# the3cloud/zktls

Hardware: AMD Instinct MI355X
Metric: trace-cells/s (higher is better)
Workload: dtype u32

## Files before the change

### zktls_amd/csrc/kernels.h

```cpp
#pragma once
#include <hip/hip_runtime.h>
#include <stddef.h>
#include <stdint.h>

#include "babybear.cuh"

namespace zk {

struct NttPassArgs {
    const uint32_t* in;
    uint32_t* out;
    uint64_t in_ld, out_ld;
    uint32_t ncols;
    uint32_t num_tiles;
    uint32_t log_m;
    uint64_t in_tile_mul, in_stride;
    uint64_t out_tile_mul, out_stride;
    uint32_t bitrev_out;
    uint32_t map_mode;
    uint64_t tile_perm;
    uint32_t fast_path;
    uint32_t debug_flags;
    uint32_t cols_per_thread;
    uint32_t bench_tag;
    const uint32_t* w1024;
    const uint32_t* pre;
    const uint32_t* post;
};
hipError_t launch_ntt_pass(const NttPassArgs& a, bool inverse, hipStream_t s);

constexpr int FUSED_COSETS = 2;
struct LdeFusedArgs {
    const uint32_t* in;
    uint64_t in_ld, out_ld;
    uint32_t ncols;
    uint32_t num_tiles;
    uint32_t map_rot;
    uint32_t grid;
    uint32_t bench_tag;
    uint64_t in_tile_mul, in_stride;
    uint64_t out_tile_mul, out_stride;
    const uint32_t* w1024_inv;
    const uint32_t* w1024_fwd;
    uint32_t* out[FUSED_COSETS];
    const uint32_t* pre[FUSED_COSETS];
    const uint32_t* post[FUSED_COSETS];
};
hipError_t launch_lde_fused(const LdeFusedArgs& a, hipStream_t s);
hipError_t launch_fused_table(uint32_t* out, const uint32_t* in, uint32_t blocks, int mode, hipStream_t s);
bool lde_fused_supported(const LdeFusedArgs& a);

struct LdeSmallArgs {
    const uint32_t* in;
    uint64_t in_ld, out_ld;
    uint32_t ncols;
    uint32_t cosets;
    uint32_t groups;
    uint32_t reserved;
    const uint32_t* tw_inv;
    const uint32_t* tw_fwd;
    uint32_t* out[16];
    const uint32_t* pre[16];
};
bool lde_small_supported(const LdeSmallArgs& a, int log_n);
hipError_t launch_lde_small(const LdeSmallArgs& a, int log_n, hipStream_t s);

struct ColPassArgs {
    const uint32_t* in;
    uint32_t* out;
    uint64_t in_batch, out_batch;
    uint32_t count;
    uint32_t tload, tstore, in_brev, out_brev;
    const uint32_t* w1024;
    const uint32_t* pre;
    const uint32_t* post2d;
};
hipError_t launch_ntt_colpass(const ColPassArgs& a, bool inverse, hipStream_t s);
hipError_t launch_post2d_table(uint32_t* out, uint32_t w, uint32_t shift, uint32_t scale, hipStream_t s);

struct CombineArgs {
    const uint32_t* in;
    uint32_t* out;
    uint64_t in_ld, out_ld;
    uint32_t ncols;
    uint64_t groups;
    int log_r;
    uint64_t in_group_mul, in_elem_mul, out_group_mul, out_elem_mul;
    int bitrev_out;
    int inverse;
    const uint32_t* tw;
};
hipError_t launch_ntt_combine(const CombineArgs& a, hipStream_t s);
hipError_t launch_combine_table(uint32_t* out, uint32_t rows, uint64_t groups, uint32_t w, uint32_t shift, uint32_t scale, int bits, hipStream_t s);

hipError_t launch_pow_table(uint32_t* out, size_t n, uint32_t base, uint32_t scale, hipStream_t s);
hipError_t launch_post_table(uint32_t* out, uint32_t rows, uint32_t cols, uint32_t omega,
                             uint32_t shift, uint32_t scale, hipStream_t s);

struct MatDesc {
    const uint32_t* ptr;
    uint64_t ld;
    uint32_t width;
};
constexpr int MAX_LEAF_MATS = 8;
constexpr uint32_t COOP_MAX_NODES = 16384;
uint32_t coop_max_nodes();
constexpr uint32_t COOP_TOP_NODES = 512;
struct LeafArgs {
    MatDesc mats[MAX_LEAF_MATS];
    int nmats;
    uint64_t height;
    uint32_t* digests;
};
hipError_t launch_hash_rows(const LeafArgs& a, hipStream_t s);
hipError_t launch_compress_level(const uint32_t* children, uint32_t* parents, uint64_t count,
                                 hipStream_t s);
hipError_t launch_inject(uint32_t* nodes, const uint32_t* extra, uint64_t count, hipStream_t s);
bool compress_inject_ok(const LeafArgs& a);
hipError_t launch_compress_inject(const uint32_t* children, const LeafArgs& a, hipStream_t s);
hipError_t launch_compress_top(uint32_t* tree, uint32_t count, hipStream_t s);
hipError_t launch_compress_sub(uint32_t* tree, uint32_t count, uint32_t sub, hipStream_t s);
hipError_t launch_hash_sub(const LeafArgs& a, uint32_t sub, hipStream_t s);
hipError_t launch_merkle_p24_colmajor(const uint32_t* mat, uint32_t cols, int log_rows, uint32_t* tree, hipStream_t s);
hipError_t launch_merkle_p24_rowmajor(const uint32_t* mat, uint64_t ld, uint32_t width, int log_rows, uint32_t* tree, hipStream_t s);
struct P2Tables;
hipError_t hash_upload_p2_tables(const P2Tables& t, hipStream_t s);
hipError_t stark_upload_p2_tables(const P2Tables& t, hipStream_t s);
namespace p2chip { struct MerkleTraceArgs; struct LayerPathsArgs; struct P2RArgs; struct MrecChainArgs; struct Fri16TranscriptArgs; }
hipError_t launch_p2chip_merkle(const p2chip::MerkleTraceArgs& a, hipStream_t s);
namespace p24chip { struct MerkleTraceArgs; struct LayerPathsArgs; struct RowPathsArgs; }
hipError_t launch_p24chip_merkle(const p24chip::MerkleTraceArgs& a, hipStream_t s);
hipError_t launch_p24chip_row_paths(const p24chip::RowPathsArgs& a, hipStream_t s);
hipError_t launch_p24chip_layer_paths(const p24chip::LayerPathsArgs& a, hipStream_t s);
hipError_t launch_fri16_transcript(const p2chip::Fri16TranscriptArgs& a, hipStream_t s);
hipError_t launch_p2chip_layer_paths(const p2chip::LayerPathsArgs& a, hipStream_t s);
hipError_t launch_mrec_chains(const p2chip::MrecChainArgs& a, hipStream_t s);
hipError_t launch_p2r_rows(const p2chip::P2RArgs& a, hipStream_t s);
hipError_t launch_permute_states(uint32_t* states, uint64_t count, hipStream_t s);

hipError_t launch_fill_uniform(uint32_t* out, uint64_t ld, uint64_t seed, uint64_t rows,
                               uint32_t width, hipStream_t s);
hipError_t launch_gen_trace(uint32_t* out, uint64_t ld, uint64_t seed, uint64_t rows,
                            uint32_t width, hipStream_t s);
hipError_t launch_gen_trace_logup(uint32_t* out, uint64_t ld, uint64_t seed, uint64_t rows, uint32_t width, uint32_t pairs,
                                  uint64_t recv_seed, uint32_t recv_width, hipStream_t s);
hipError_t launch_small_eval(const uint32_t* in, uint64_t in_ld, uint32_t* out, uint64_t out_ld, int log_n, int log_out, uint32_t width,
                             uint32_t w, uint32_t shift, uint32_t scale, int bitrev_out, hipStream_t s);
hipError_t launch_transpose(const uint32_t* in, uint32_t* out, uint64_t rows, uint64_t cols, int rev_bits_in, int rev_bits_out, hipStream_t s);
hipError_t launch_convert(const uint32_t* in, uint32_t* out, uint64_t n, bool to_monty_form,
                          hipStream_t s);

hipError_t launch_domain_tables(uint32_t* xs, uint32_t* sel_first, uint32_t* sel_last, uint32_t* itw, int log_n, int log_blowup, hipStream_t s);

struct QuotientArgs {
    const uint32_t* lde;
    uint64_t ld;
    uint32_t width;
    int log_n;
    int lanes_per_row;
    const uint32_t* xs;
    const uint32_t* sel_first;
    uint32_t wn_inv;
    uint32_t inv_zh_even, inv_zh_odd;
    const uint32_t* alpha_pow;
    uint32_t pairs;
    const uint32_t* perm;
    uint64_t perm_ld;
    Ext gamma, beta;
    Ext cumsum;
    const uint32_t* sel_last;
    uint32_t* addend_out;
    const uint32_t* addend;
    uint32_t* out;
    uint32_t* lde_out;
    uint64_t lde_ld;
};
hipError_t launch_quotient(const QuotientArgs& a, hipStream_t s);
hipError_t launch_logup_addend(const QuotientArgs& a, hipStream_t s);

constexpr uint32_t AIR_SLOT_EXTRA = 4;
constexpr uint32_t AIR_GP = 36;
#if defined(__HIPCC__)
__host__ __device__
#endif
inline uint32_t air_lds_base(uint32_t slot, uint32_t W) {
    if (slot < W) return AIR_GP * (slot >> 2) + (slot & 3u);
    if (slot < 2 * W) { const uint32_t c = slot - W; return AIR_GP * (c >> 2) + (c & 3u) + 4u; }
    const uint32_t x = slot - 2 * W;
    return AIR_GP * ((W >> 2) + (x >> 2)) + (x & 3u);
}
struct QuotientAirArgs {
    const uint32_t* lde; uint64_t ld; uint32_t width; int log_n;
    const uint32_t* xs; const uint32_t* sel_first; const uint32_t* sel_last;
    uint32_t wn_inv;
    int log_qd;
    uint32_t inv_zh[4];
    const uint32_t* body;
    uint32_t n_constraints;
    const uint32_t* weights;
    const uint32_t* pub;
    uint32_t* out;
    uint32_t* lde_out; uint64_t lde_ld;
    const uint32_t* recs; uint32_t n_terms; uint32_t n_public;
    const uint32_t* addend;
    uint32_t no_chain;
    uint32_t wide;
    uint32_t cls[6];
};
constexpr uint32_t AIR_WIDE_POINTS = 64, AIR_WIDE_PITCH = 65;
inline bool air_wide_form(uint32_t width, uint32_t n_terms, int log_n, uint32_t n_public) {
    return n_terms >= 2048 && width % 4 == 0 && (size_t)AIR_WIDE_PITCH * (width + AIR_SLOT_EXTRA + n_public) * 4 <= 160 * 1024 && log_n >= 6;
}
ZK_HD uint32_t air_wide_word(uint32_t slot, uint32_t W) {
    if (slot < W) return AIR_WIDE_PITCH * slot;
    if (slot < 2 * W) return AIR_WIDE_PITCH * (slot - W) + 1u;
    return AIR_WIDE_PITCH * (W + (slot - 2 * W));
}
hipError_t launch_quotient_air(const QuotientAirArgs& a, hipStream_t s);

hipError_t launch_inv_denominators(const uint32_t* xs, uint64_t count, const Ext& z0, const Ext& z1, int npoints,
                                   uint32_t* out, uint32_t* xw, uint64_t xw_count, hipStream_t s);

struct OpenArgs {
    const uint32_t* mat;
    uint64_t ld;
    uint32_t width;
    uint64_t rows;
    const uint32_t* xw;
    uint64_t xw_stride;
    uint32_t* partial;
    int tx;
};
size_t open_chunks(uint64_t rows, uint32_t width, uint64_t ld, const uint32_t* mat);
hipError_t launch_open(const OpenArgs& a, int npts, const Ext& scale0, const Ext& scale1, uint32_t* out, hipStream_t s);

struct ReducedArgs {
    const uint32_t* tlde; uint64_t t_ld; uint32_t width;
    const uint32_t* qlde; uint64_t q_ld; uint32_t q_width;
    const uint32_t* plde; uint64_t p_ld; uint32_t p_width;
    uint64_t rows;
    const uint32_t* alpha_pow;
    const uint32_t* dinv;
    Ext y_loc, y_next, y_pl, y_pn, y_q, off_next, off_pl, off_pn, off_q;
    Ext off_loc;
    int accumulate;
    uint32_t* out;
};
hipError_t launch_reduced_opening(const ReducedArgs& a, uint32_t* scratch_at, hipStream_t s);
int rowdot_form(uint32_t width, uint64_t rows);

struct PermArgs {
    const uint32_t* trace; uint64_t ld;
    uint64_t rows; uint32_t pairs;
    Ext gamma, beta;
    uint32_t* out; uint64_t out_ld;
};
hipError_t launch_perm_trace(const PermArgs& a, uint32_t* block_scratch, hipStream_t s);

constexpr int LOOKUP_REC_WORDS = 12;
struct LookupArgs {
    const uint32_t* table; uint32_t ni, cols;
    Ext gamma, bpow[9];
    const uint8_t* cmap; uint32_t n_used, chunk_mask;
};
constexpr uint32_t LOOKUP_MAX_COLS = 512, LOOKUP_STAGE_MAX_USED = 56;
struct MachinePermArgs {
    LookupArgs lk;
    const uint32_t* trace; uint64_t ld; uint64_t rows;
    uint32_t* out; uint64_t out_ld;
    const uint32_t* pre; uint64_t pre_ld; uint32_t pre_w;
};
bool lookup_perm_two_sources_ok(const MachinePermArgs& a);
hipError_t launch_perm_trace_machine(const MachinePermArgs& a, uint32_t* block_scratch, hipStream_t s);
struct MachineQuotArgs {
    LookupArgs lk;
    const uint32_t* lde; uint64_t ld; const uint32_t* perm; uint64_t perm_ld; int log_n;
    int log_qd;
    const uint32_t* xs; const uint32_t* sel_first; const uint32_t* sel_last; uint32_t wn_inv;
    const uint32_t* weights;
    Ext cumsum;
    uint32_t* addend;
};
hipError_t launch_lookup_addend(const MachineQuotArgs& a, hipStream_t s);

hipError_t launch_fri_fold(const uint32_t* in, uint32_t* out, const uint32_t* itw, uint64_t half, const Ext& beta, hipStream_t s);
hipError_t launch_ext_add(uint32_t* dst, const uint32_t* src, uint64_t count, hipStream_t s);
hipError_t launch_fri_fold_dev(const uint32_t* in, uint32_t* out, const uint32_t* itw, uint64_t half, const uint32_t* beta_ptr,
                               int squarings, hipStream_t s);

struct DevChallenger {
    uint32_t state[16];
    uint32_t in[8];
    uint32_t out[8];
    int32_t n_in, n_out;
};
hipError_t launch_fri_challenge(DevChallenger* chal, const uint32_t* root, uint32_t* beta_out, uint32_t* root_log, hipStream_t s);


struct GrindArgs {
    uint32_t state[16];
    int slot;
    uint32_t mask;
};
hipError_t launch_grind(const GrindArgs& a, uint32_t base, uint32_t count, uint32_t* result, hipStream_t s);

struct GatherDesc {
    const uint32_t* src;
    uint32_t dst_off;
    uint32_t nwords;
};
hipError_t launch_gather(const GatherDesc* descs, uint32_t ndesc, uint32_t* dst, hipStream_t s);

hipError_t launch_copy_bytes(void* dst, const void* src, size_t bytes, hipStream_t s);
hipError_t launch_fill_bytes(void* dst, int byte, size_t bytes, hipStream_t s);
hipError_t launch_copy2d(uint32_t* dst, uint64_t dst_ld, const uint32_t* src, uint64_t src_ld, uint32_t width, uint64_t rows, hipStream_t s);
}
```

### zktls_amd/csrc/prover.cpp

```cpp
#include <atomic>
#include <chrono>
#include <condition_variable>
#include <deque>
#include <cstring>
#include <functional>
#include <mutex>
#include <string>
#include <thread>
#include <vector>

#include "proof_common.h"
#include "batch.h"

namespace zk { std::atomic<bool> g_fri_graph{true}; }
namespace zk {

extern std::atomic<uint64_t> g_p2_generation;
void air_digest_cached(const AirView& a, uint32_t out[8]) {
    struct Entry { std::vector<uint32_t> words; uint64_t generation; uint32_t dg[8]; };
    static std::mutex mu;
    static std::vector<Entry> cache;
    const uint64_t gen = g_p2_generation.load();
    {
        std::lock_guard<std::mutex> lk(mu);
        for (const Entry& e : cache)
            if (e.generation == gen && e.words.size() == a.words && memcmp(e.words.data(), a.w, a.words * 4) == 0) { memcpy(out, e.dg, 32); return; }
    }
    air_digest(a, out);
    std::lock_guard<std::mutex> lk(mu);
    if (cache.size() >= 64) cache.erase(cache.begin());
    Entry e;
    e.words.assign(a.w, a.w + a.words);
    e.generation = gen;
    memcpy(e.dg, out, 32);
    cache.push_back(std::move(e));
}

static int ensure_domain(zkhip_ctx* ctx, int log_n, int log_blowup = 1) {
    if (ctx->dom_log_n == log_n && ctx->dom_log_blowup == log_blowup) return ZKHIP_OK;
    for (const auto& d : ctx->domains)
        if (d.log_n == log_n && d.log_blowup == log_blowup) {
            ctx->dom_xs = d.xs; ctx->dom_sel_first = d.sel_first; ctx->dom_sel_last = d.sel_last; ctx->dom_itw = d.itw;
            ctx->dom_log_n = log_n; ctx->dom_log_blowup = log_blowup;
            return ZKHIP_OK;
        }
    zkhip_ctx::DomainSet d{log_n, log_blowup, nullptr, nullptr, nullptr, nullptr};
    const size_t m = (size_t)1 << (log_n + log_blowup), mq = (size_t)1 << (log_n + (log_blowup < 2 ? log_blowup : 2));
    ZK_HIP(hipMalloc((void**)&d.xs, m * 4));
    ZK_HIP(hipMalloc((void**)&d.sel_first, mq * 4));
    ZK_HIP(hipMalloc((void**)&d.sel_last, mq * 4));
    ZK_HIP(hipMalloc((void**)&d.itw, (m / 2) * 4));
    ZK_HIP(launch_domain_tables(d.xs, d.sel_first, d.sel_last, d.itw, log_n, log_blowup, ctx->stream));
    ctx->domains.push_back(d);
    ctx->dom_xs = d.xs; ctx->dom_sel_first = d.sel_first; ctx->dom_sel_last = d.sel_last; ctx->dom_itw = d.itw;
    ctx->dom_log_n = log_n; ctx->dom_log_blowup = log_blowup;
    return ZKHIP_OK;
}
static int ensure_fold_table(zkhip_ctx* ctx, int log_h) {
    if (ctx->dom_log_n >= 0 && ctx->dom_log_n + ctx->dom_log_blowup >= log_h) return ZKHIP_OK;
    return ensure_domain(ctx, log_h - 1 < 5 ? 5 : log_h - 1, 1);
}

static int d2h(zkhip_ctx* ctx, void* dst, const void* src, size_t bytes) { return dev_d2h(ctx, dst, src, bytes); }
static int h2d(zkhip_ctx* ctx, void* dst, const void* src, size_t bytes) { return dev_h2d(ctx, dst, src, bytes); }

struct LogupIn {
    Ext cumsum = ext_zero();
    uint32_t pairs = 0;
    const uint32_t* perm_lde = nullptr;
    Ext gamma = ext_zero(), beta = ext_zero();
};
static int run_quotient(zkhip_ctx* ctx, const uint32_t* lde, size_t ld, int log_n, uint32_t width, const Ext& alpha,
                        const LogupIn& lu, uint32_t* out_chunks, uint32_t* lde_out = nullptr, size_t lde_ld = 0) {
    if (ctx->dom_log_n != log_n) ZK_TRY(ensure_domain(ctx, log_n));
    const uint32_t G = width / 4;
    const size_t K = (size_t)3 * G + (lu.pairs ? lu.pairs + 3 : 0);
    std::vector<Ext> ap(K);
    Ext w = ext_one();
    for (size_t k = K; k-- > 0;) { ap[k] = w; w = ext_mul(w, alpha); }
    std::vector<uint32_t> tab(16 * (size_t)G + 4 * (K - 3 * (size_t)G));
    for (uint32_t g = 0; g < G; g++) {
        for (int t = 0; t < 3; t++) memcpy(&tab[16 * (size_t)g + 4 * t], ap[3 * (size_t)g + t].c, 16);
        tab[16 * (size_t)g + 12] = to_monty(g + 1);
        tab[16 * (size_t)g + 13] = to_monty(2 * g + 3);
        tab[16 * (size_t)g + 14] = to_monty(5 * g + 7);
        tab[16 * (size_t)g + 15] = 0;
    }
    for (size_t k = 3 * (size_t)G; k < K; k++) memcpy(&tab[16 * (size_t)G + 4 * (k - 3 * (size_t)G)], ap[k].c, 16);
    void* d_ap;
    ZK_TRY(ctx_reserve(ctx, S_APOW_Q, tab.size() * 4, &d_ap));
    ZK_TRY(h2d(ctx, d_ap, tab.data(), tab.size() * 4));
    QuotientArgs q{};
    q.lde = lde; q.ld = ld; q.width = width; q.log_n = log_n;
    q.lanes_per_row = pow2ceil((int)G) > 16 ? 16 : pow2ceil((int)G);
    q.xs = ctx->dom_xs; q.sel_first = ctx->dom_sel_first;
    q.wn_inv = finv(two_adic_generator(log_n));
    const uint32_t gn = fpow(MONTY_GEN, (uint64_t)1 << log_n);
    q.inv_zh_even = finv(fsub(gn, MONTY_R1));
    q.inv_zh_odd = finv(fsub(fneg(gn), MONTY_R1));
    q.alpha_pow = (const uint32_t*)d_ap;
    q.pairs = lu.pairs; q.perm = lu.perm_lde; q.perm_ld = 4 * ((uint64_t)lu.pairs + 1);
    q.gamma = lu.gamma; q.beta = lu.beta; q.cumsum = lu.cumsum; q.sel_last = ctx->dom_sel_last;
    q.out = out_chunks;
    q.lde_out = lde_out; q.lde_ld = lde_ld;
    if (lu.pairs) {
        void* v_add;
        ZK_TRY(ctx_reserve(ctx, S_ADDEND, ((size_t)2 << log_n) * 16, &v_add));
        q.addend_out = (uint32_t*)v_add;
        ZK_HIP(launch_logup_addend(q, ctx->stream));
        q.addend = (const uint32_t*)v_add;
    }
    ZK_HIP(launch_quotient(q, ctx->stream));
    return ZKHIP_OK;
}

static int run_quotient_air(zkhip_ctx* ctx, const AirView& air, const uint32_t* lde, size_t ld, int log_n, uint32_t width,
                            const uint32_t* public_values, const Ext& alpha, uint32_t* out_chunks, uint32_t* lde_out, size_t lde_ld,
                            const Ext& scale = ext_one(), const uint32_t* addend = nullptr) {
    if (ctx->dom_log_n != log_n || ctx->dom_log_blowup < air.lqd) ZK_TRY(ensure_domain(ctx, log_n, air.lqd));
    std::vector<uint32_t> body, weights;
    air_device_image(air, alpha, body, weights, scale);
    std::vector<uint32_t> pub(air.n_public ? air.n_public : 1, 0u);
    for (uint32_t i = 0; i < air.n_public; i++) pub[i] = to_monty(public_values[i]);
    std::vector<uint32_t> recs;
    uint32_t cls[6] = {0, 0, 0, 0, 0, 0};
    const bool wide = !t_batcher && ld % 4 == 0 && (reinterpret_cast<uintptr_t>(lde) & 15u) == 0 &&
                      air_wide_form(width, (uint32_t)air_term_count(air), log_n, 0);
    if (wide) air_term_records_wide(air, alpha, pub.data(), recs, cls, scale);
    else air_term_records(air, alpha, pub.data(), recs, scale);
    const size_t body_w = (body.size() + 3) & ~(size_t)3, pub_w = (pub.size() + 3) & ~(size_t)3;
    std::vector<uint32_t> stage(body_w + weights.size() + pub_w + recs.size(), 0u);
    memcpy(stage.data(), body.data(), body.size() * 4);
    memcpy(stage.data() + body_w, weights.data(), weights.size() * 4);
    memcpy(stage.data() + body_w + weights.size(), pub.data(), pub.size() * 4);
    if (!recs.empty()) memcpy(stage.data() + body_w + weights.size() + pub_w, recs.data(), recs.size() * 4);
    void* d_stage;
    ZK_TRY(ctx_reserve(ctx, S_APOW_Q, stage.size() * 4, &d_stage));
    ZK_TRY(h2d(ctx, d_stage, stage.data(), stage.size() * 4));
    QuotientAirArgs q{};
    q.lde = lde; q.ld = ld; q.width = width; q.log_n = log_n;
    q.xs = ctx->dom_xs; q.sel_first = ctx->dom_sel_first; q.sel_last = ctx->dom_sel_last;
    q.wn_inv = finv(two_adic_generator(log_n));
    q.log_qd = air.lqd;
    const uint32_t gn = fpow(MONTY_GEN, (uint64_t)1 << log_n), wq = two_adic_generator(air.lqd);
    for (int j = 0; j < (1 << air.lqd); j++) q.inv_zh[j] = finv(fsub(fmul(gn, fpow(wq, (uint64_t)j)), MONTY_R1));
    q.body = (const uint32_t*)d_stage; q.n_constraints = air.K;
    q.weights = (const uint32_t*)d_stage + body_w; q.pub = (const uint32_t*)d_stage + body_w + weights.size();
    q.out = out_chunks; q.lde_out = lde_out; q.lde_ld = lde_ld;
    q.recs = recs.empty() ? nullptr : (const uint32_t*)d_stage + body_w + weights.size() + pub_w;
    q.n_terms = (uint32_t)(recs.size() / 8); q.n_public = recs.empty() ? air.n_public : 0u;
    q.wide = wide ? 1u : 0u;
    for (int i = 0; i < 6; i++) q.cls[i] = cls[i];
    q.addend = addend;
    ZK_HIP(launch_quotient_air(q, ctx->stream));
    return ZKHIP_OK;
}

static int run_open(zkhip_ctx* ctx, const uint32_t* lde, size_t ld, int log_n, uint32_t width, const Ext* z, int npts,
                    const uint32_t* xw, uint32_t* d_out) {
    const uint64_t n = (uint64_t)1 << log_n;
    OpenArgs o{};
    o.mat = lde; o.ld = ld; o.width = width; o.rows = n; o.xw = xw; o.xw_stride = n;
    o.tx = pow2ceil((int)width) > 64 ? 64 : pow2ceil((int)width);
    const size_t nchunks = open_chunks(n, width, ld, lde);
    void* part;
    ZK_TRY(ctx_reserve(ctx, S_PARTIAL, nchunks * npts * width * 16, &part));
    o.partial = (uint32_t*)part;
    Ext scale[2] = {ext_zero(), ext_zero()};
    const uint32_t ginv = finv(MONTY_GEN), ninv = finv(to_monty((uint32_t)(n % P)));
    for (int k = 0; k < npts; k++)
        scale[k] = ext_mul_base(ext_sub_base(ext_pow(ext_mul_base(z[k], ginv), n), MONTY_R1), ninv);
    ZK_HIP(launch_open(o, npts, scale[0], scale[1], d_out, ctx->stream));
    return ZKHIP_OK;
}

static int commit_hw(zkhip_ctx* ctx, const uint32_t* mat, size_t ld, uint32_t width, int log_h, uint32_t* tree, int hw) {
    if (hw == 24) { ZK_HIP(launch_merkle_p24_rowmajor(mat, ld, width, log_h, tree, ctx->stream)); return ZKHIP_OK; }
    MatDesc md{mat, ld, width};
    return op_merkle_commit(ctx, &md, 1, log_h, tree);
}

static int fri_commit_phase(zkhip_ctx* ctx, Challenger& ch, const Shape& sh, int H, int RL, uint32_t* layers, uint32_t* ltrees,
                            const std::vector<size_t>& layer_off, const std::vector<size_t>& tree_off, uint32_t* fold_tmp, size_t m,
                            const uint32_t* const* inject, uint32_t* pf, size_t& pos) {
    hipStream_t st = ctx->stream;
    const int K = sh.K;
    const size_t arity = (size_t)1 << K;
    uint32_t root[8];
#ifdef ZKHIP_AB_HOOKS
    static const bool fri_on_host = [] { const char* e = getenv("ZKHIP_FRI_HOST"); return e && atoi(e) != 0; }();
#else
    constexpr bool fri_on_host = false;
#endif
    void* v_chal = nullptr;
    uint32_t *d_betas = nullptr, *d_roots = nullptr;
    DevChallenger* d_chal = nullptr;
    if (!fri_on_host && RL > 0) {
        ZK_TRY(ctx_reserve(ctx, S_CHAL, sizeof(DevChallenger) + (size_t)RL * 12 * 4, &v_chal));
        d_chal = (DevChallenger*)v_chal;
        d_betas = (uint32_t*)((char*)v_chal + sizeof(DevChallenger));
        d_roots = d_betas + 4 * (size_t)RL;
        DevChallenger hc{};
        for (int i = 0; i < 16; i++) hc.state[i] = ch.state[i];
        for (int i = 0; i < 8; i++) { hc.in[i] = ch.in[i]; hc.out[i] = ch.out[i]; }
        hc.n_in = ch.n_in; hc.n_out = ch.n_out;
        ZK_TRY(h2d(ctx, d_chal, &hc, sizeof hc));
    }
    auto enqueue_layers = [&]() -> int {
    for (int l = 0; l < RL; l++) {
        const int lh = H - K * (l + 1);
        const size_t rows = (size_t)1 << lh;
        uint32_t* cur = layers + layer_off[l];
        uint32_t* tree = ltrees + tree_off[l];
        ZK_TRY(commit_hw(ctx, cur, 4 * arity, (uint32_t)(4 * arity), lh, tree, sh.hw));
        Ext beta = ext_zero();
        if (d_chal) {
            ZK_HIP(launch_fri_challenge(d_chal, tree + (2 * rows - 2) * 8, d_betas + 4 * l, d_roots + 8 * l, st));
        } else {
            ZK_TRY(d2h(ctx, root, tree + (2 * rows - 2) * 8, 32));
            for (int i = 0; i < 8; i++) { ch.observe(root[i]); pf[pos++] = from_monty(root[i]); }
            beta = ch.sample_ext();
        }
        const uint32_t* src = cur;
        for (int j = 0; j < K; j++) {
            const size_t out_cnt = (size_t)1 << (H - K * l - j - 1);
            uint32_t* dst = (j == K - 1) ? layers + layer_off[l + 1] : fold_tmp + ((j & 1) ? 4 * (m / 2) : 0);
            if (d_chal) ZK_HIP(launch_fri_fold_dev(src, dst, ctx->dom_itw, out_cnt, d_betas + 4 * l, j, st));
            else ZK_HIP(launch_fri_fold(src, dst, ctx->dom_itw, out_cnt, beta, st));
            src = dst;
            beta = ext_mul(beta, beta);
        }
        const int reached = H - K * (l + 1);
        if (inject && inject[reached]) ZK_HIP(launch_ext_add(layers + layer_off[l + 1], inject[reached], (uint64_t)1 << reached, st));
    }
    return ZKHIP_OK;
    };
#ifdef ZKHIP_AB_HOOKS
    static const bool env_graph = [] { const char* e = getenv("ZKHIP_FRI_GRAPH"); return !e || atoi(e) != 0; }();
    const bool use_graph = env_graph && g_fri_graph.load();
#else
    const bool use_graph = g_fri_graph.load();
#endif
    if (d_chal && use_graph && !t_batcher) {
        std::vector<uint64_t> key = {(uint64_t)H, (uint64_t)K, (uint64_t)RL, (uint64_t)sh.hw, (uint64_t)m, (uint64_t)(uintptr_t)layers,
                                     (uint64_t)(uintptr_t)ltrees, (uint64_t)(uintptr_t)fold_tmp, (uint64_t)(uintptr_t)d_chal,
                                     (uint64_t)(uintptr_t)ctx->dom_itw};
        for (size_t o : layer_off) key.push_back(o);
        for (size_t o : tree_off) key.push_back(o);
        if (inject) for (int h = 0; h <= H; h++) key.push_back((uint64_t)(uintptr_t)inject[h]);
        if (!ctx->fri_graph_exec || ctx->fri_graph_key != key) {
            if (ctx->fri_graph_exec) { (void)hipGraphExecDestroy(ctx->fri_graph_exec); ctx->fri_graph_exec = nullptr; }
            hipGraph_t graph = nullptr;
            ZK_HIP(hipStreamBeginCapture(st, hipStreamCaptureModeThreadLocal));
// ... 1240 lines not shown
```

### zktls_amd/csrc/stark.hip

```cpp
#include <atomic>

#include "poseidon2.cuh"
#include "kernels.h"
#include "batch.h"

namespace zk {

hipError_t stark_upload_p2_tables(const P2Tables& t, hipStream_t s) { return p2_upload_tables(t, s); }


ZK_D Ext ld_ext(const uint32_t* p) {
    uint4 v = *reinterpret_cast<const uint4*>(p);
    return Ext{{v.x, v.y, v.z, v.w}};
}
ZK_D void st_ext(uint32_t* p, const Ext& e) { *reinterpret_cast<uint4*>(p) = make_uint4(e.c[0], e.c[1], e.c[2], e.c[3]); }

ZK_D Ext group_sum(Ext v, int width) {
    for (int off = width >> 1; off > 0; off >>= 1) {
        Ext o;
        o.c[0] = __shfl_down(v.c[0], off, width);
        o.c[1] = __shfl_down(v.c[1], off, width);
        o.c[2] = __shfl_down(v.c[2], off, width);
        o.c[3] = __shfl_down(v.c[3], off, width);
        v = Ext{{dadd(v.c[0], o.c[0]), dadd(v.c[1], o.c[1]), dadd(v.c[2], o.c[2]), dadd(v.c[3], o.c[3])}};
    }
    return v;
}

__device__ __forceinline__ void domain_tables_kernel_body(uint32_t* xs, uint32_t* sel_first, uint32_t* sel_last, uint32_t* itw, int log_n, int log_blowup, uint32_t g_pow_n) {
    const uint32_t p = blockIdx.x * blockDim.x + threadIdx.x;
    const int H = log_n + log_blowup, lq = log_blowup < 2 ? log_blowup : 2, Hq = log_n + lq;
    if (p >= (1u << H)) return;
    const uint32_t e = __brev(p) >> (32 - H);
    const uint32_t wm = two_adic_generator(H);
    const uint32_t x = fmul(MONTY_GEN, fpow(wm, e));
    xs[p] = x;
    if (p < (1u << Hq)) {
        const uint32_t eq = __brev(p) >> (32 - Hq);
        const uint32_t xn = fmul(g_pow_n, fpow(two_adic_generator(lq), eq & ((1u << lq) - 1u)));
        const uint32_t zh = fsub(xn, MONTY_R1);
        sel_first[p] = fmul(zh, finv(fsub(x, MONTY_R1)));
        sel_last[p] = fmul(zh, finv(fsub(x, finv(two_adic_generator(log_n)))));
    }
    if (p < (1u << (H - 1))) {
        const uint32_t ei = (H > 1) ? (__brev(p) >> (32 - (H - 1))) : 0u;
        itw[p] = fmul(finv(fpow(wm, ei)), MONTY_INV2);
    }
}
__global__ void domain_tables_kernel(uint32_t* xs, uint32_t* sel_first, uint32_t* sel_last, uint32_t* itw, int log_n, int log_blowup, uint32_t g_pow_n) { domain_tables_kernel_body(xs, sel_first, sel_last, itw, log_n, log_blowup, g_pow_n); }
struct domain_tables_kernel_bargs { uint32_t* xs; uint32_t* sel_first; uint32_t* sel_last; uint32_t* itw; int log_n; int log_blowup; uint32_t g_pow_n; static domain_tables_kernel_bargs make(uint32_t* xs, uint32_t* sel_first, uint32_t* sel_last, uint32_t* itw, int log_n, int log_blowup, uint32_t g_pow_n) { return domain_tables_kernel_bargs{xs, sel_first, sel_last, itw, log_n, log_blowup, g_pow_n}; } };
__global__ void domain_tables_kernel_batch(const domain_tables_kernel_bargs* __restrict__ zk_arr) { const domain_tables_kernel_bargs& zk_b = zk_arr[blockIdx.z]; domain_tables_kernel_body(zk_b.xs, zk_b.sel_first, zk_b.sel_last, zk_b.itw, zk_b.log_n, zk_b.log_blowup, zk_b.g_pow_n); }

hipError_t launch_domain_tables(uint32_t* xs, uint32_t* sel_first, uint32_t* sel_last, uint32_t* itw, int log_n, int log_blowup, hipStream_t s) {
    const uint32_t m = 1u << (log_n + log_blowup);
    const uint32_t gpn = fpow(MONTY_GEN, (uint64_t)1 << log_n);
    ZK_LAUNCH(domain_tables_kernel, domain_tables_kernel_batch, domain_tables_kernel_bargs, dim3((m + 255) / 256), dim3(256), 0, s, xs, sel_first, sel_last, itw, log_n, log_blowup, gpn);
    return hipGetLastError();
}

typedef uint32_t u32x4_nt __attribute__((ext_vector_type(4)));
ZK_D uint4 ld_stream(const uint32_t* p) {
    const u32x4_nt v = __builtin_nontemporal_load(reinterpret_cast<const u32x4_nt*>(p));
    return make_uint4(v.x, v.y, v.z, v.w);
}
ZK_D void dacc1(uint64_t& acc, uint32_t a0, uint32_t b0) {
    const uint64_t t = dmac(a0, b0, acc);
    acc = ((uint64_t)dred((uint32_t)(t >> 32)) << 32) | (uint32_t)t;
}
template <int CTRL>
ZK_D uint32_t dpp_mov(uint32_t v) { return (uint32_t)__builtin_amdgcn_update_dpp(0, (int)v, CTRL, 0xF, 0xF, false); }
ZK_D uint32_t row_group_sum(uint32_t v, int L) {
    if (L > 1) v = dadd(v, dpp_mov<0xB1>(v));
    if (L > 2) v = dadd(v, dpp_mov<0x4E>(v));
    if (L > 4) v = dadd(v, dpp_mov<0x141>(v));
    if (L > 8) v = dadd(v, dpp_mov<0x140>(v));
    return v;
}
__device__ __forceinline__ void logup_addend_kernel_body(const QuotientArgs& a) {
    const int H = a.log_n + 1;
    const uint32_t m = 1u << H;
    const uint32_t p = blockIdx.x * blockDim.x + threadIdx.x;
    if (p >= m) return;
    const uint32_t e = __brev(p) >> (32 - H);
    const uint32_t pn = __brev((e + 2) & (m - 1)) >> (32 - H);
    const uint32_t* row = a.lde + (uint64_t)p * a.ld;
    const uint32_t* prow = a.perm + (uint64_t)p * a.perm_ld;
    const uint32_t* pnrow = a.perm + (uint64_t)pn * a.perm_ld;
    const uint32_t* wl = a.alpha_pow + 16 * (a.width / 4);
    const uint32_t sel_trans = dsub(a.xs[p], a.wn_inv);
    Ext r = ext_zero(), sphi = ext_zero(), sphin = ext_zero();
    for (uint32_t q = 0; q < a.pairs; q++) {
        const uint4 vs = *reinterpret_cast<const uint4*>(row + 8 * q);
        const uint4 vr = *reinterpret_cast<const uint4*>(row + 8 * q + 4);
        const Ext ds = ext_add(ext_add_base(a.gamma, vs.x), ext_mul_base_dev(a.beta, vs.y));
        const Ext dr = ext_add(ext_add_base(a.gamma, vr.x), ext_mul_base_dev(a.beta, vr.y));
        const Ext phi = ld_ext(prow + 4 * q), phin = ld_ext(pnrow + 4 * q);
        const Ext c = ext_sub(ext_mul_dev(ext_mul_dev(phi, ds), dr), ext_sub(dr, ds));
        r = ext_add(r, ext_mul_dev(c, ld_ext(wl + 4 * q)));
        sphi = ext_add(sphi, phi);
        sphin = ext_add(sphin, phin);
    }
    const Ext S = ld_ext(prow + 4 * a.pairs), Sn = ld_ext(pnrow + 4 * a.pairs);
    const Ext F1 = ext_mul_base_dev(ld_ext(wl + 4 * a.pairs), a.sel_first[p]);
    const Ext F2 = ext_mul_base_dev(ld_ext(wl + 4 * (a.pairs + 1)), sel_trans);
    const Ext F3 = ext_mul_base_dev(ld_ext(wl + 4 * (a.pairs + 2)), a.sel_last[p]);
    r = ext_add(r, ext_mul_dev(F1, ext_sub(S, sphi)));
    r = ext_add(r, ext_mul_dev(F2, ext_sub(ext_sub(Sn, S), sphin)));
    r = ext_add(r, ext_mul_dev(F3, ext_sub(S, a.cumsum)));
    st_ext(a.addend_out + 4 * (uint64_t)p, r);
}
__global__ void __launch_bounds__(256) logup_addend_kernel(QuotientArgs a) { logup_addend_kernel_body(a); }
struct logup_addend_kernel_bargs { QuotientArgs a; static logup_addend_kernel_bargs make(QuotientArgs a) { return logup_addend_kernel_bargs{a}; } };
__global__ void __launch_bounds__(256) logup_addend_kernel_batch(const logup_addend_kernel_bargs* __restrict__ zk_arr) { const logup_addend_kernel_bargs& zk_b = zk_arr[blockIdx.z]; logup_addend_kernel_body(zk_b.a); }

hipError_t launch_logup_addend(const QuotientArgs& a, hipStream_t s) {
    const uint64_t m = 2ull << a.log_n;
    ZK_LAUNCH(logup_addend_kernel, logup_addend_kernel_batch, logup_addend_kernel_bargs, dim3((unsigned)((m + 255) / 256)), dim3(256), 0, s, a);
    return hipGetLastError();
}
constexpr int QCHAIN = 16;
template <int NG>
#ifndef QWPE
#define QWPE 2
#endif
__device__ __forceinline__ void quotient_kernel_body(const QuotientArgs& a) {
    const int L = a.lanes_per_row;
    const uint32_t gid = blockIdx.x * blockDim.x + threadIdx.x;
    const int lane = gid % L;
    const int H = a.log_n + 1;
    const uint32_t m = 1u << H;
    const uint32_t nchains = m / QCHAIN;
    const bool live = gid / L < nchains;
    const uint32_t chain = live ? gid / L : 0u;
    const uint32_t parity = chain & 1u;
    uint32_t e = 2u * ((chain >> 1) * QCHAIN) + parity;
    const uint32_t G = a.width / 4;
    const uint32_t inv_zh = parity ? a.inv_zh_odd : a.inv_zh_even;

    uint4 cur[NG], nxt[NG];
    uint32_t p = __brev(e) >> (32 - H);
#pragma unroll
    for (int t = 0; t < NG; t++) {
        const uint32_t g = lane + L * t;
        cur[t] = g < G ? *reinterpret_cast<const uint4*>(a.lde + (uint64_t)p * a.ld + 4 * g) : make_uint4(0, 0, 0, 0);
    }
    constexpr bool HOIST = NG <= 4;
    uint4 W[HOIST ? NG : 1][4];
    if (HOIST) {
#pragma unroll
        for (int t = 0; t < NG; t++) {
            const uint32_t g = lane + L * t;
            const uint4* wp = reinterpret_cast<const uint4*>(a.alpha_pow + 16 * (g < G ? g : 0u));
#pragma unroll
            for (int i = 0; i < 4; i++) W[HOIST ? t : 0][i] = wp[i];
        }
    }
    for (int step = 0; step < QCHAIN; step++) {
        const uint32_t en = (e + 2) & (m - 1);
        const uint32_t pn = __brev(en) >> (32 - H);
#pragma unroll
        for (int t = 0; t < NG; t++) {
            const uint32_t g = lane + L * t;
            nxt[t] = g < G ? ld_stream(a.lde + (uint64_t)pn * a.ld + 4 * g) : make_uint4(0, 0, 0, 0);
        }
        const uint32_t x = a.xs[p];
        const uint32_t sel_first = a.sel_first[p];
        const uint32_t sel_trans = dsub(x, a.wn_inv);
        uint64_t acc[4] = {0, 0, 0, 0};
#pragma unroll
        for (int t = 0; t < NG; t++) {
            const uint32_t g = lane + L * t;
            if (g < G) {
                const uint4 v = cur[t];
                const uint4* wp = reinterpret_cast<const uint4*>(a.alpha_pow + 16 * g);
                const uint4 w0 = HOIST ? W[HOIST ? t : 0][0] : wp[0], w1 = HOIST ? W[HOIST ? t : 0][1] : wp[1];
                const uint4 w2 = HOIST ? W[HOIST ? t : 0][2] : wp[2], kk = HOIST ? W[HOIST ? t : 0][3] : wp[3];
                const uint32_t aab = dmul(dmont_lazy(v.x, v.x), v.y);
                const uint32_t c1 = dsub(dsub(v.z, aab), kk.x);
                const uint32_t ab = dmul(v.x, v.y);
                const uint32_t c2 = dmul(dsub_lazy(dsub(dsub(nxt[t].w, ab), v.z), kk.y), sel_trans);
                const uint32_t c3 = dmul(dsub_lazy(v.w, kk.z), sel_first);
                dacc2(acc[0], w0.x, c1, w1.x, c2); dacc1(acc[0], w2.x, c3);
                dacc2(acc[1], w0.y, c1, w1.y, c2); dacc1(acc[1], w2.y, c3);
                dacc2(acc[2], w0.z, c1, w1.z, c2); dacc1(acc[2], w2.z, c3);
                dacc2(acc[3], w0.w, c1, w1.w, c2); dacc1(acc[3], w2.w, c3);
            }
        }
        Ext r = Ext{{dacc_finish(acc[0]), dacc_finish(acc[1]), dacc_finish(acc[2]), dacc_finish(acc[3])}};
        if (a.addend && lane == 0) r = ext_add(r, ld_ext(a.addend + 4 * (uint64_t)p));
#pragma unroll
        for (int i = 0; i < 4; i++) r.c[i] = row_group_sum(r.c[i], L);
        if (lane == 0 && live) {
            r = ext_mul_base_dev(r, inv_zh);
            st_ext(a.out + ((uint64_t)parity * (m >> 1) + (e >> 1)) * 4, r);
            if (a.lde_out) st_ext(a.lde_out + (uint64_t)p * a.lde_ld + 4u * parity, r);
        }
#pragma unroll
        for (int t = 0; t < NG; t++) cur[t] = nxt[t];
        e = en; p = pn;
    }
}
template <int NG>
#ifndef QWPE
#define QWPE 2
#endif
__global__ void __launch_bounds__(256) __attribute__((amdgpu_waves_per_eu(QWPE, QWPE))) quotient_kernel(QuotientArgs a) { quotient_kernel_body<NG>(a); }
struct quotient_kernel_bargs { QuotientArgs a; static quotient_kernel_bargs make(QuotientArgs a) { return quotient_kernel_bargs{a}; } };
template <int NG>
#ifndef QWPE
#define QWPE 2
#endif
__global__ void __launch_bounds__(256) __attribute__((amdgpu_waves_per_eu(QWPE, QWPE))) quotient_kernel_batch(const quotient_kernel_bargs* __restrict__ zk_arr) { const quotient_kernel_bargs& zk_b = zk_arr[blockIdx.z]; quotient_kernel_body<NG>(zk_b.a); }

constexpr int SLICE_COLS = 32;
constexpr int SLICE_PITCH = SLICE_COLS + 4;
constexpr uint64_t STREAM_MIN_ROWS = 2048;
ZK_D void wave_lds_handover() {
    __builtin_amdgcn_fence(__ATOMIC_RELEASE, "wavefront");
    __builtin_amdgcn_wave_barrier();
    __builtin_amdgcn_fence(__ATOMIC_ACQUIRE, "wavefront");
}
#ifdef ZKHIP_AB_HOOKS
static bool stream_forms_off() { const char* e = getenv("ZKHIP_STREAM_OLD"); return e && atoi(e) != 0; }
#endif

__device__ __forceinline__ void quotient_stream_kernel_body(const QuotientArgs& a) {
    __shared__ __attribute__((aligned(16))) uint32_t tile[4][65 * SLICE_PITCH];
    const uint32_t lane = threadIdx.x & 63u, wave = threadIdx.x >> 6;
    const int H = a.log_n + 1;
    const uint32_t m = 1u << H;
    const uint32_t wpp = m >> 7;
    const uint32_t gw = blockIdx.x * 4u + wave;
    if (gw >= 2u * wpp) return;
    const uint32_t parity = gw / wpp, j0 = (gw % wpp) * 64u;
    uint32_t* t = tile[wave];
    const uint32_t part = lane & 7u, sub = lane >> 3;
    const uint32_t* src[9];
#pragma unroll
    for (int k = 0; k < 9; k++) {
        const uint32_t j = j0 + 8u * k + (k < 8 ? sub : 0u);
        const uint32_t pr = __brev((2u * j + parity) & (m - 1)) >> (32 - H);
        src[k] = a.lde + (uint64_t)pr * a.ld + 4u * part;
    }
    const bool tail = lane < 8u;
    uint4 pf[9];
#pragma unroll
    for (int k = 0; k < 8; k++) pf[k] = ld_stream(src[k]);
    pf[8] = tail ? ld_stream(src[8]) : make_uint4(0, 0, 0, 0);

    const uint32_t j = j0 + lane;
    const uint32_t p = __brev(2u * j + parity) >> (32 - H);
    uint32_t sel_first = a.sel_first[p];
    const uint32_t sel_trans = dsub(a.xs[p], a.wn_inv);
    asm("" : "+v"(sel_first));
    const uint32_t nsl = a.width / SLICE_COLS;
    uint64_t acc[4] = {0, 0, 0, 0};
    for (uint32_t s = 0; s < nsl; s++) {
#pragma unroll
        for (int k = 0; k < 8; k++) *reinterpret_cast<uint4*>(t + (8u * k + sub) * SLICE_PITCH + 4u * part) = pf[k];
        if (tail) *reinterpret_cast<uint4*>(t + 64u * SLICE_PITCH + 4u * part) = pf[8];
        if (s + 1 < nsl) {
#pragma unroll
            for (int k = 0; k < 8; k++) pf[k] = ld_stream(src[k] + SLICE_COLS * (s + 1));
            if (tail) pf[8] = ld_stream(src[8] + SLICE_COLS * (s + 1));
        }
        wave_lds_handover();
        const uint4* wp = reinterpret_cast<const uint4*>(a.alpha_pow + 16u * (SLICE_COLS / 4) * s);
#pragma unroll
        for (int g = 0; g < SLICE_COLS / 4; g++) {
            const uint4 v = *reinterpret_cast<const uint4*>(t + lane * SLICE_PITCH + 4 * g);
            const uint32_t dn = t[(lane + 1u) * SLICE_PITCH + 4 * g + 3];
            const uint4 w0 = wp[4 * g], w1 = wp[4 * g + 1], w2 = wp[4 * g + 2], kk = wp[4 * g + 3];
            const uint32_t aab = dmul(dmont_lazy(v.x, v.x), v.y);
            const uint32_t c1 = dsub(dsub(v.z, aab), kk.x);
            const uint32_t ab = dmul(v.x, v.y);
            const uint32_t c2 = dmul(dsub_lazy(dsub(dsub(dn, ab), v.z), kk.y), sel_trans);
            const uint32_t c3 = dmul(dsub_lazy(v.w, kk.z), sel_first);
            dacc2(acc[0], w0.x, c1, w1.x, c2); dacc1(acc[0], w2.x, c3);
            dacc2(acc[1], w0.y, c1, w1.y, c2); dacc1(acc[1], w2.y, c3);
            dacc2(acc[2], w0.z, c1, w1.z, c2); dacc1(acc[2], w2.z, c3);
            dacc2(acc[3], w0.w, c1, w1.w, c2); dacc1(acc[3], w2.w, c3);
        }
        wave_lds_handover();
    }
    Ext r = Ext{{dacc_finish(acc[0]), dacc_finish(acc[1]), dacc_finish(acc[2]), dacc_finish(acc[3])}};
    if (a.addend) r = ext_add(r, ld_ext(a.addend + 4 * (uint64_t)p));
    r = ext_mul_base_dev(r, parity ? a.inv_zh_odd : a.inv_zh_even);
    st_ext(a.out + ((uint64_t)parity * (m >> 1) + j) * 4, r);
    if (a.lde_out) st_ext(a.lde_out + (uint64_t)p * a.lde_ld + 4u * parity, r);
}
__global__ void __launch_bounds__(256) quotient_stream_kernel(QuotientArgs a) { quotient_stream_kernel_body(a); }
struct quotient_stream_kernel_bargs { QuotientArgs a; static quotient_stream_kernel_bargs make(QuotientArgs a) { return quotient_stream_kernel_bargs{a}; } };
__global__ void __launch_bounds__(256) quotient_stream_kernel_batch(const quotient_stream_kernel_bargs* __restrict__ zk_arr) { const quotient_stream_kernel_bargs& zk_b = zk_arr[blockIdx.z]; quotient_stream_kernel_body(zk_b.a); }

static bool quotient_stream_form(const QuotientArgs& a) {
#ifdef ZKHIP_AB_HOOKS
    if (stream_forms_off()) return false;
#endif
    return a.width % SLICE_COLS == 0 && (2ull << a.log_n) >= STREAM_MIN_ROWS;
}

hipError_t launch_quotient(const QuotientArgs& a, hipStream_t s) {
    const uint64_t m = 2ull << a.log_n;
    if (quotient_stream_form(a)) {
        ZK_LAUNCH(quotient_stream_kernel, quotient_stream_kernel_batch, quotient_stream_kernel_bargs, dim3((unsigned)(m / 256)), dim3(256), 0, s, a);
        return hipGetLastError();
    }
    const uint64_t threads = (m / QCHAIN) * a.lanes_per_row;
    const uint32_t G = a.width / 4;
    const int ng = (int)((G + a.lanes_per_row - 1) / a.lanes_per_row);
    const dim3 grid((unsigned)((threads + 255) / 256)), block(256);
    switch (ng) {
        case 1: ZK_LAUNCH(quotient_kernel<1>, quotient_kernel_batch<1>, quotient_kernel_bargs, grid, block, 0, s, a); break;
        case 2: ZK_LAUNCH(quotient_kernel<2>, quotient_kernel_batch<2>, quotient_kernel_bargs, grid, block, 0, s, a); break;
        case 3: ZK_LAUNCH(quotient_kernel<3>, quotient_kernel_batch<3>, quotient_kernel_bargs, grid, block, 0, s, a); break;
        case 4: ZK_LAUNCH(quotient_kernel<4>, quotient_kernel_batch<4>, quotient_kernel_bargs, grid, block, 0, s, a); break;
        case 5: case 6: case 7: case 8: ZK_LAUNCH(quotient_kernel<8>, quotient_kernel_batch<8>, quotient_kernel_bargs, grid, block, 0, s, a); break;
        default: ZK_LAUNCH(quotient_kernel<16>, quotient_kernel_batch<16>, quotient_kernel_bargs, grid, block, 0, s, a); break;
    }
    return hipGetLastError();
}

__device__ __forceinline__ void quotient_air_kernel_body(const QuotientAirArgs& a) {
    const int H = a.log_n + a.log_qd;
    const uint32_t m = 1u << H, nq = 1u << a.log_qd;
    const uint32_t p = blockIdx.x * blockDim.x + threadIdx.x;
    if (p >= m) return;
    const uint32_t e = __brev(p) >> (32 - H);
    const uint32_t pn = __brev((e + nq) & (m - 1)) >> (32 - H);
    const uint32_t* local = a.lde + (uint64_t)p * a.ld;
    const uint32_t* next = a.lde + (uint64_t)pn * a.ld;
    const uint32_t x = a.xs[p];
    const uint32_t sel_first = a.sel_first[p], sel_last = a.sel_last[p], sel_trans = dsub(x, a.wn_inv);
    uint64_t acc[4] = {0, 0, 0, 0};
    const uint32_t* w = a.body;
    for (uint32_t k = 0; k < a.n_constraints; k++) {
        const uint32_t sel = *w++, nt = *w++;
        uint32_t c = 0;
        for (uint32_t t = 0; t < nt; t++) {
            uint32_t prod = *w++;
            const uint32_t d = *w++;
            for (uint32_t j = 0; j < d; j++) {
                const uint32_t v = *w++, kind = v >> 30, idx = v & 0xFFFFu;
                const uint32_t val = kind == 0 ? local[idx] : (kind == 1 ? next[idx] : a.pub[idx]);
                prod = dmul(prod, val);
            }
            c = dadd(c, prod);
        }
        if (sel) c = dmul(c, sel == 1 ? sel_first : (sel == 2 ? sel_last : sel_trans));
        const uint4 wt = *reinterpret_cast<const uint4*>(a.weights + 4 * (uint64_t)k);
        dacc1(acc[0], wt.x, c); dacc1(acc[1], wt.y, c); dacc1(acc[2], wt.z, c); dacc1(acc[3], wt.w, c);
    }
    const uint32_t chunk = e & (nq - 1u);
    Ext r = Ext{{dacc_finish(acc[0]), dacc_finish(acc[1]), dacc_finish(acc[2]), dacc_finish(acc[3])}};
    if (a.addend) r = ext_add(r, ld_ext(a.addend + 4 * (uint64_t)p));
    const uint32_t iz = chunk == 0 ? a.inv_zh[0] : (chunk == 1 ? a.inv_zh[1] : (chunk == 2 ? a.inv_zh[2] : a.inv_zh[3]));
    r = ext_mul_base_dev(r, iz);
    st_ext(a.out + ((uint64_t)chunk * (m >> a.log_qd) + (e >> a.log_qd)) * 4, r);
    if (a.lde_out) st_ext(a.lde_out + (uint64_t)p * a.lde_ld + 4u * chunk, r);
}
__global__ void __launch_bounds__(256) quotient_air_kernel(QuotientAirArgs a) { quotient_air_kernel_body(a); }
struct quotient_air_kernel_bargs { QuotientAirArgs a; static quotient_air_kernel_bargs make(QuotientAirArgs a) { return quotient_air_kernel_bargs{a}; } };
__global__ void __launch_bounds__(256) quotient_air_kernel_batch(const quotient_air_kernel_bargs* __restrict__ zk_arr) { const quotient_air_kernel_bargs& zk_b = zk_arr[blockIdx.z]; quotient_air_kernel_body(zk_b.a); }

__device__ __forceinline__ uint32_t air_group_e0(const QuotientAirArgs& a, uint32_t g) { return ((g >> a.log_qd) * 8u << a.log_qd) + (g & ((1u << a.log_qd) - 1u)); }
__device__ __forceinline__ uint32_t air_row_of(const QuotientAirArgs& a, uint32_t e0, uint32_t r) {
    const int H = a.log_n + a.log_qd;
    return __brev((e0 + (r << a.log_qd)) & ((1u << H) - 1u)) >> (32 - H);
}
__device__ __forceinline__ void air_load8(const uint32_t* slots, uint32_t base, uint32_t (&v)[8]) {
    const uint32_t* b = slots + base;
#pragma unroll
    for (int q = 0; q < 8; q++) v[q] = b[4 * q];
}
template <int NT>
__device__ __forceinline__ void air_stage_extras(const QuotientAirArgs& a, uint32_t* slots, uint32_t e0, uint32_t tid) {
    const uint32_t W4 = a.width >> 2;
    if (tid < 8) {
        const uint32_t p = air_row_of(a, e0, tid);
        const uint4 ex = {a.sel_first[p], a.sel_last[p], dsub(a.xs[p], a.wn_inv), MONTY_R1};
        *reinterpret_cast<uint4*>(slots + AIR_GP * W4 + 4u * tid) = ex;
    }
    for (uint32_t i = tid >> 3; i < a.n_public; i += NT / 8) slots[air_lds_base(2 * a.width + AIR_SLOT_EXTRA + i, a.width) + 4u * (tid & 7u)] = a.pub[i];
}
__device__ __forceinline__ void air_store_point(const QuotientAirArgs& a, uint32_t e, Ext r) {
    const int H = a.log_n + a.log_qd;
    const uint32_t m = 1u << H, nq = 1u << a.log_qd;
    const uint32_t p = __brev(e) >> (32 - H);
    if (a.addend) r = ext_add(r, ld_ext(a.addend + 4 * (uint64_t)p));
    const uint32_t chunk = e & (nq - 1u);
    const uint32_t iz = chunk == 0 ? a.inv_zh[0] : (chunk == 1 ? a.inv_zh[1] : (chunk == 2 ? a.inv_zh[2] : a.inv_zh[3]));
    r = ext_mul_base_dev(r, iz);
    st_ext(a.out + ((uint64_t)chunk * (m >> a.log_qd) + (e >> a.log_qd)) * 4, r);
    if (a.lde_out) st_ext(a.lde_out + (uint64_t)p * a.lde_ld + 4u * chunk, r);
}
template <int NT>
__device__ __forceinline__ void quotient_air_terms_kernel_body(const QuotientAirArgs& a) {
    constexpr int PTS = 8;
    static_assert(NT == 64 || NT == 128 || NT == 256, "one, two or four wavefronts per group");
    extern __shared__ uint32_t slots[];
    const uint32_t tid = threadIdx.x, W4 = a.width >> 2;
    const uint32_t mask = (1u << (a.log_n + a.log_qd)) - 1u;
    const uint32_t e0 = air_group_e0(a, blockIdx.x);
#pragma unroll
    for (int r = 0; r < 9; r++) {
        const uint4* row = reinterpret_cast<const uint4*>(a.lde + (uint64_t)air_row_of(a, e0, r) * a.ld);
        for (uint32_t cg = tid; cg < W4; cg += NT) *reinterpret_cast<uint4*>(slots + AIR_GP * cg + 4u * r) = row[cg];
    }
    air_stage_extras<NT>(a, slots, e0, tid);
    __syncthreads();
    uint64_t acc[PTS][4];
#pragma unroll
    for (int q = 0; q < PTS; q++)
#pragma unroll
        for (int i = 0; i < 4; i++) acc[q][i] = 0;
    const uint4* recs = reinterpret_cast<const uint4*>(a.recs);
    auto load8 = [&](uint32_t o, uint32_t (&v)[PTS]) { air_load8(slots, o, v); };
    auto product = [&](const uint4& o, uint32_t (&prod)[PTS]) {
        const uint32_t n = o.z >> 16;
        uint32_t v[PTS];
        load8(o.x & 0xFFFFu, prod);
        const uint32_t offs[4] = {o.x >> 16, o.y & 0xFFFFu, o.y >> 16, o.z & 0xFFFFu};
        for (uint32_t k = 1; k < n; k++) {
            load8(offs[k - 1], v);
#pragma unroll
            for (int q = 0; q < PTS; q++) prod[q] = dmul(prod[q], v[q]);
        }
    };
    for (uint32_t t = 2 * tid; t < a.n_terms; t += 2 * NT) {
        const uint4 ca = recs[2 * (size_t)t], oa = recs[2 * (size_t)t + 1], cb = recs[2 * (size_t)t + 2], ob = recs[2 * (size_t)t + 3];
        uint32_t pa[PTS], pb[PTS];
        product(oa, pa);
        product(ob, pb);
#pragma unroll
        for (int q = 0; q < PTS; q++) {
            dacc2(acc[q][0], ca.x, pa[q], cb.x, pb[q]); dacc2(acc[q][1], ca.y, pa[q], cb.y, pb[q]);
            dacc2(acc[q][2], ca.z, pa[q], cb.z, pb[q]); dacc2(acc[q][3], ca.w, pa[q], cb.w, pb[q]);
        }
// ... 1101 lines not shown
```

Baseline: 21.68 billion.

## Factor constant and selector terms out of quotient inner loop

The quotient stream kernel now keeps three separate per-constraint accumulators. The per-group constants are summed on the host (K1..K3), and sel_trans and sel_first are multiplied once per row at the end rather than once per column group. This removes two multiplies and several subtractions from the inner loop. It also changes how rows are mapped to lanes: each lane handles strided rows, so the next-row value comes from a neighbouring lane's row or from a compact tail buffer, and the tail row is loaded by all lanes. In exchange it uses more accumulator registers and a more complex row-index mapping.

```diff
diff --git a/zktls_amd/csrc/kernels.h b/zktls_amd/csrc/kernels.h
--- a/zktls_amd/csrc/kernels.h
+++ b/zktls_amd/csrc/kernels.h
@@ -163,6 +163,7 @@
     uint32_t wn_inv;
     uint32_t inv_zh_even, inv_zh_odd;
     const uint32_t* alpha_pow;
+    Ext K1, K2, K3;
     uint32_t pairs;
     const uint32_t* perm;
     uint64_t perm_ld;
diff --git a/zktls_amd/csrc/prover.cpp b/zktls_amd/csrc/prover.cpp
--- a/zktls_amd/csrc/prover.cpp
+++ b/zktls_amd/csrc/prover.cpp
@@ -79,7 +79,10 @@
     Ext w = ext_one();
     for (size_t k = K; k-- > 0;) { ap[k] = w; w = ext_mul(w, alpha); }
     std::vector<uint32_t> tab(16 * (size_t)G + 4 * (K - 3 * (size_t)G));
+    Ext kf[3] = {ext_zero(), ext_zero(), ext_zero()};
     for (uint32_t g = 0; g < G; g++) {
+        const uint32_t kg[3] = {to_monty(g + 1), to_monty(2 * g + 3), to_monty(5 * g + 7)};
+        for (int t = 0; t < 3; t++) kf[t] = ext_add(kf[t], ext_mul_base(ap[3 * (size_t)g + t], kg[t]));
         for (int t = 0; t < 3; t++) memcpy(&tab[16 * (size_t)g + 4 * t], ap[3 * (size_t)g + t].c, 16);
         tab[16 * (size_t)g + 12] = to_monty(g + 1);
         tab[16 * (size_t)g + 13] = to_monty(2 * g + 3);
@@ -99,6 +102,7 @@
     q.inv_zh_even = finv(fsub(gn, MONTY_R1));
     q.inv_zh_odd = finv(fsub(fneg(gn), MONTY_R1));
     q.alpha_pow = (const uint32_t*)d_ap;
+    q.K1 = kf[0]; q.K2 = kf[1]; q.K3 = kf[2];
     q.pairs = lu.pairs; q.perm = lu.perm_lde; q.perm_ld = 4 * ((uint64_t)lu.pairs + 1);
     q.gamma = lu.gamma; q.beta = lu.beta; q.cumsum = lu.cumsum; q.sel_last = ctx->dom_sel_last;
     q.out = out_chunks;
diff --git a/zktls_amd/csrc/stark.hip b/zktls_amd/csrc/stark.hip
--- a/zktls_amd/csrc/stark.hip
+++ b/zktls_amd/csrc/stark.hip
@@ -66,6 +66,14 @@
 ZK_D void dacc1(uint64_t& acc, uint32_t a0, uint32_t b0) {
     const uint64_t t = dmac(a0, b0, acc);
     acc = ((uint64_t)dred((uint32_t)(t >> 32)) << 32) | (uint32_t)t;
+}
+struct QTerms { uint32_t c1, c2, c3; };
+ZK_D QTerms quotient_terms(const uint4& v, uint32_t dn) {
+    const uint32_t ab = dmul(v.x, v.y);
+    return QTerms{dsub(v.z, dmul(v.x, ab)), dsub(dsub(dn, ab), v.z), v.w};
+}
+ZK_D void qacc2(uint64_t (&s)[4], const uint4& wa, uint32_t ca, const uint4& wb, uint32_t cb) {
+    dacc2(s[0], wa.x, ca, wb.x, cb); dacc2(s[1], wa.y, ca, wb.y, cb); dacc2(s[2], wa.z, ca, wb.z, cb); dacc2(s[3], wa.w, ca, wb.w, cb);
 }
 template <int CTRL>
 ZK_D uint32_t dpp_mov(uint32_t v) { return (uint32_t)__builtin_amdgcn_update_dpp(0, (int)v, CTRL, 0xF, 0xF, false); }
@@ -225,65 +233,69 @@
 #endif
 
 __device__ __forceinline__ void quotient_stream_kernel_body(const QuotientArgs& a) {
-    __shared__ __attribute__((aligned(16))) uint32_t tile[4][65 * SLICE_PITCH];
+    constexpr uint32_t TAIL = 64u * SLICE_PITCH;
+    __shared__ __attribute__((aligned(16))) uint32_t tile[4][TAIL + 64u];
     const uint32_t lane = threadIdx.x & 63u, wave = threadIdx.x >> 6;
     const int H = a.log_n + 1;
     const uint32_t m = 1u << H;
     const uint32_t wpp = m >> 7;
     const uint32_t gw = blockIdx.x * 4u + wave;
     if (gw >= 2u * wpp) return;
-    const uint32_t parity = gw / wpp, j0 = (gw % wpp) * 64u;
+    const uint32_t parity = gw / wpp, e0 = 16u * (gw % wpp) + parity;
     uint32_t* t = tile[wave];
     const uint32_t part = lane & 7u, sub = lane >> 3;
     const uint32_t* src[9];
 #pragma unroll
-    for (int k = 0; k < 9; k++) {
-        const uint32_t j = j0 + 8u * k + (k < 8 ? sub : 0u);
-        const uint32_t pr = __brev((2u * j + parity) & (m - 1)) >> (32 - H);
-        src[k] = a.lde + (uint64_t)pr * a.ld + 4u * part;
-    }
-    const bool tail = lane < 8u;
+    for (int i = 0; i < 9; i++) {
+        const uint32_t pr = __brev(((sub << (H - 3)) + e0 + 2u * i) & (m - 1)) >> (32 - H);
+        src[i] = a.lde + (uint64_t)pr * a.ld + 4u * part;
+    }
     uint4 pf[9];
 #pragma unroll
-    for (int k = 0; k < 8; k++) pf[k] = ld_stream(src[k]);
-    pf[8] = tail ? ld_stream(src[8]) : make_uint4(0, 0, 0, 0);
-
-    const uint32_t j = j0 + lane;
-    const uint32_t p = __brev(2u * j + parity) >> (32 - H);
+    for (int i = 0; i < 9; i++) pf[i] = ld_stream(src[i]);
+
+    const uint32_t e = ((lane & 7u) << (H - 3)) + e0 + 2u * (lane >> 3);
+    const uint32_t j = e >> 1;
+    const uint32_t p = __brev(e) >> (32 - H);
+    const uint32_t dn_at = lane < 56u ? (lane + 8u) * SLICE_PITCH + 3u : TAIL + 8u * (lane & 7u);
+    const uint32_t dn_step = lane < 56u ? 4u : 1u;
     uint32_t sel_first = a.sel_first[p];
     const uint32_t sel_trans = dsub(a.xs[p], a.wn_inv);
     asm("" : "+v"(sel_first));
     const uint32_t nsl = a.width / SLICE_COLS;
-    uint64_t acc[4] = {0, 0, 0, 0};
+    uint64_t s1[4] = {0, 0, 0, 0}, s2[4] = {0, 0, 0, 0}, s3[4] = {0, 0, 0, 0};
     for (uint32_t s = 0; s < nsl; s++) {
 #pragma unroll
-        for (int k = 0; k < 8; k++) *reinterpret_cast<uint4*>(t + (8u * k + sub) * SLICE_PITCH + 4u * part) = pf[k];
-        if (tail) *reinterpret_cast<uint4*>(t + 64u * SLICE_PITCH + 4u * part) = pf[8];
+        for (int i = 0; i < 8; i++) *reinterpret_cast<uint4*>(t + (8u * i + sub) * SLICE_PITCH + 4u * part) = pf[i];
+        t[TAIL + lane] = pf[8].w;
         if (s + 1 < nsl) {
 #pragma unroll
-            for (int k = 0; k < 8; k++) pf[k] = ld_stream(src[k] + SLICE_COLS * (s + 1));
-            if (tail) pf[8] = ld_stream(src[8] + SLICE_COLS * (s + 1));
+            for (int i = 0; i < 9; i++) pf[i] = ld_stream(src[i] + SLICE_COLS * (s + 1));
         }
         wave_lds_handover();
         const uint4* wp = reinterpret_cast<const uint4*>(a.alpha_pow + 16u * (SLICE_COLS / 4) * s);
 #pragma unroll
-        for (int g = 0; g < SLICE_COLS / 4; g++) {
-            const uint4 v = *reinterpret_cast<const uint4*>(t + lane * SLICE_PITCH + 4 * g);
-            const uint32_t dn = t[(lane + 1u) * SLICE_PITCH + 4 * g + 3];
-            const uint4 w0 = wp[4 * g], w1 = wp[4 * g + 1], w2 = wp[4 * g + 2], kk = wp[4 * g + 3];
-            const uint32_t aab = dmul(dmont_lazy(v.x, v.x), v.y);
-            const uint32_t c1 = dsub(dsub(v.z, aab), kk.x);
-            const uint32_t ab = dmul(v.x, v.y);
-            const uint32_t c2 = dmul(dsub_lazy(dsub(dsub(dn, ab), v.z), kk.y), sel_trans);
-            const uint32_t c3 = dmul(dsub_lazy(v.w, kk.z), sel_first);
-            dacc2(acc[0], w0.x, c1, w1.x, c2); dacc1(acc[0], w2.x, c3);
-            dacc2(acc[1], w0.y, c1, w1.y, c2); dacc1(acc[1], w2.y, c3);
-            dacc2(acc[2], w0.z, c1, w1.z, c2); dacc1(acc[2], w2.z, c3);
-            dacc2(acc[3], w0.w, c1, w1.w, c2); dacc1(acc[3], w2.w, c3);
+        for (int g = 0; g < SLICE_COLS / 4; g += 2) {
+            const uint4 va = *reinterpret_cast<const uint4*>(t + lane * SLICE_PITCH + 4 * g);
+            const uint4 vb = *reinterpret_cast<const uint4*>(t + lane * SLICE_PITCH + 4 * g + 4);
+            const QTerms ca = quotient_terms(va, t[dn_at + g * dn_step]);
+            const QTerms cb = quotient_terms(vb, t[dn_at + (g + 1) * dn_step]);
+            const uint4* wa = wp + 4 * g;
+            const uint4* wb = wp + 4 * g + 4;
+            qacc2(s1, wa[0], ca.c1, wb[0], cb.c1);
+            qacc2(s2, wa[1], ca.c2, wb[1], cb.c2);
+            qacc2(s3, wa[2], ca.c3, wb[2], cb.c3);
         }
         wave_lds_handover();
     }
-    Ext r = Ext{{dacc_finish(acc[0]), dacc_finish(acc[1]), dacc_finish(acc[2]), dacc_finish(acc[3])}};
+    Ext r;
+#pragma unroll
+    for (int i = 0; i < 4; i++) {
+        const uint32_t r1 = dsub(dacc_finish(s1[i]), a.K1.c[i]);
+        const uint32_t r2 = dmul(dsub(dacc_finish(s2[i]), a.K2.c[i]), sel_trans);
+        const uint32_t r3 = dmul(dsub(dacc_finish(s3[i]), a.K3.c[i]), sel_first);
+        r.c[i] = dadd(dadd(r1, r2), r3);
+    }
     if (a.addend) r = ext_add(r, ld_ext(a.addend + 4 * (uint64_t)p));
     r = ext_mul_base_dev(r, parity ? a.inv_zh_odd : a.inv_zh_even);
     st_ext(a.out + ((uint64_t)parity * (m >> 1) + j) * 4, r);
```

After: 21.84 billion (median of 6 runs). Within noise of the previous version (+0.7%).
